# abhi1kumar/SUP-NeRF

Hardware: AMD Instinct MI355X
Metric: rays/sec at 4096 rays x 64 samples (fused render forward) (higher is better)
Workload: dtype f32

## Files before the change

### sup-nerf_amd/csrc/snr_mlp16.hip

```cpp
#include <atomic>

#include "snr_mlp16_core.hpp"
#include "snr_host.hpp"

namespace snr {

struct Epi {
    float lo;
    const float* zlds;
    const float* zglb;
    float hi;
    float* dump;
};
struct EpiRegs { f32x4 z; };

__device__ __forceinline__ uint32_t spread_nibbles(uint32_t m16) {
    return ((m16 >> 12) & 0xFu) | (((m16 >> 8) & 0xFu) << 8) | (((m16 >> 4) & 0xFu) << 16) | ((m16 & 0xFu) << 24);
}

template <bool LATLDS>
__device__ __forceinline__ EpiRegs epi_load(const Epi& c, int T, int g) {
    EpiRegs e;
    e.z = f32x4{0.f, 0.f, 0.f, 0.f};
    if (LATLDS) e.z = *reinterpret_cast<const f32x4*>(c.zlds + 16 * T + 4 * g);
    else if (c.zglb) e.z = *reinterpret_cast<const f32x4*>(c.zglb + 16 * T + 4 * g);
    return e;
}

template <bool MASKS>
__device__ __forceinline__ void epi_value(const f32x4& acc, f32x4& x, const Epi& c, const EpiRegs& e, int r, uint32_t& m16) {
    float v = acc[r];
    if (MASKS) m16 = __builtin_amdgcn_alignbit(m16, __float_as_uint(0.f - v), 31);
    v = __builtin_amdgcn_fmed3f(v, c.lo, c.hi);
    x[r] = v + e.z[r];
    if (MASKS) asm volatile("" : "+v"(m16));
}

template <int NT>
__device__ __forceinline__ void acc_from_bias(f32x4 (&acc)[16], const float* bias , int g) {
#pragma unroll
    for (int t = 0; t < NT; ++t) acc[t] = *reinterpret_cast<const f32x4*>(bias + 16 * t + 4 * g);
}

template <int NT, int WAVES, bool LATLDS, bool MASKS, bool DUMP>
__device__ __forceinline__ void layer_from_acc(f32x4 (&accP)[16], Ring16& ring, float* lds, const float* bias, const Epi& c, int g, const Dma16& dm,
                                               const float* base, bool pre, const f32x4 (&xe)[2], const float* next_first, int next_rows,
                                               uint32_t (&mw)[4]) {
    f32x4 accC[16];
    f32x4 a0, a1;
    constexpr int rows_mid = NT * 16;
    constexpr int chunk_floats = rows_mid * KC;
    if (pre) {
        chunk_dma16<WAVES>(dm, base, lds + (ring.cur ^ 1) * WBUF16, lds, rows_mid);
        const float* wb = lds + ring.cur * WBUF16;
        first_pair(a0, a1, wb + ring.aoff[0]);
        acc_from_bias<NT>(accC, bias, g);
        tile_mma<NT, false>(accC, accP, xe[0], wb + ring.aoff[0], a0, a1, wb + ring.aoff[1]);
        tile_mma<NT, false>(accC, accP, xe[1], wb + ring.aoff[1], a0, a1, nullptr);
        ring_turn(ring);
    } else {
        acc_from_bias<NT>(accC, bias, g);
    }
    constexpr int NG = NT / 2;
    EpiRegs e = epi_load<LATLDS>(c, 0, g);
    f32x4 xa, xb;
    uint32_t m16 = 0u;
#pragma unroll
    for (int r = 3; r >= 0; --r) epi_value<MASKS>(accP[0], xa, c, e, r, m16);
    if (DUMP) *reinterpret_cast<f32x4*>(c.dump) = xa;
#pragma unroll
    for (int ch = 0; ch < 8; ++ch) {
        const float* src = (ch < 7) ? base + (ch + 1) * chunk_floats : next_first;
        const int rows = (ch < 7) ? rows_mid : next_rows;
        float* const dst = lds + (ring.cur ^ 1) * WBUF16;
        const float* wb = lds + ring.cur * WBUF16;
        first_pair(a0, a1, wb + ring.aoff[0]);
        tile_mma<NT, false>(accC, accP, xa, wb + ring.aoff[0], a0, a1, wb + ring.aoff[1], [&](int gi) {
            if (gi == 0) e = epi_load<LATLDS>(c, 2 * ch + 1, g);
            constexpr int PSTEP = (WAVES == 8) ? 2 : 1;
            if (gi % PSTEP == 0 && (gi / PSTEP) * 8 * WAVES < rows) chunk_piece16<WAVES>(dm, src, dst, lds, rows, gi / PSTEP);
#pragma unroll
            for (int k = (gi * 4) / NG; k < ((gi + 1) * 4) / NG; ++k) epi_value<MASKS>(accP[2 * ch + 1], xb, c, e, 3 - k, m16);
            if (DUMP && gi == NG - 1) *reinterpret_cast<f32x4*>(c.dump + 16 * (2 * ch + 1)) = xb;
        });
        if (ch & 1) { mw[ch >> 1] = m16; m16 = 0u; }
        if (ch == 7) {
            tile_mma<NT, true>(accC, accP, xb, wb + ring.aoff[1], a0, a1, nullptr);
        } else {
            tile_mma<NT, false>(accC, accP, xb, wb + ring.aoff[1], a0, a1, nullptr, [&](int gi) {
                if (gi == 0) e = epi_load<LATLDS>(c, 2 * ch + 2, g);
#pragma unroll
                for (int k = (gi * 4) / NG; k < ((gi + 1) * 4) / NG; ++k) epi_value<MASKS>(accP[2 * ch + 2], xa, c, e, 3 - k, m16);
                if (DUMP && gi == NG - 1) *reinterpret_cast<f32x4*>(c.dump + 16 * (2 * ch + 2)) = xa;
            });
        }
        ring_turn(ring);
    }
}

__device__ __forceinline__ void store_masks16x4(uint4* __restrict__ dst , const uint32_t (&mw)[4], int wave, int lane) {
    const int n = lane & 15, g = lane >> 4;
    uint32_t w[4];
#pragma unroll
    for (int i = 0; i < 4; ++i) {
        const uint32_t mine = spread_nibbles(mw[i]) << (4 * (g >> 1));
        w[i] = mine | (uint32_t)__shfl_xor((int)mine, 32, 64);
    }
    if (g < 2) dst[16 * (wave & 1) + n + 32 * g] = make_uint4(w[0], w[1], w[2], w[3]);
}

#ifdef SNR_STAMPS
#define SNR16_STAMP(i) do { if (io.sigmas && lane == 0) { unsigned long long t_; asm volatile("s_memtime %0\n\ts_waitcnt lgkmcnt(0)" : "=s"(t_) :: "memory"); \
        reinterpret_cast<unsigned long long*>(io.sigmas)[(tile_wg * WAVES + wave) * 8 + (i)] = t_; } } while (0)
#define SNR16_STAMP_HWID(i) do { if (io.sigmas && lane == 0) { unsigned a_, b_; asm volatile("s_getreg_b32 %0, hwreg(HW_REG_HW_ID)\n\ts_getreg_b32 %1, hwreg(HW_REG_XCC_ID)" : "=s"(a_), "=s"(b_)); \
        reinterpret_cast<unsigned long long*>(io.sigmas)[(tile_wg * WAVES + wave) * 8 + (i)] = (unsigned long long)a_ | ((unsigned long long)b_ << 32); } } while (0)
#else
#define SNR16_STAMP(i) do {} while (0)
#define SNR16_STAMP_HWID(i) do {} while (0)
#endif

template <int MODE> struct PointSrc { using T = RayGeom; };
template <> struct PointSrc<3> { using T = snr_lattice; };
struct BrickSrc {
    snr_lattice lat;
    const int* bricks;
    long long n_objects;
};
template <> struct PointSrc<4> { using T = BrickSrc; };

template <int MODE, int WAVES, bool LATLDS, bool MASKS, bool DUMP>
__global__ void __launch_bounds__(WAVES * 64, 2)
decoder_fwd16_kernel(DecoderIO io, Layout L, Lds16 lo, const float* __restrict__ xyz, const float* __restrict__ viewdir, typename PointSrc<MODE>::T gm,
                     float* __restrict__ out_rgb, float* __restrict__ out_depth, float* __restrict__ out_acc) {
    extern __shared__ __attribute__((aligned(16))) float lds[];
    constexpr int WGP = WAVES * 16;
    constexpr bool DENS = MODE >= 2;
    const int tid = threadIdx.x, lane = tid & 63, wave = tid >> 6, n = lane & 15, g = lane >> 4;
    const long long tile_wg = blockIdx.x;
    const long long gp_raw = tile_wg * WGP + wave * 16 + n;
    const bool live = gp_raw < io.n_points;
    const long long gp = live ? gp_raw : io.n_points - 1;
    const long long tile32 = tile_wg * (WAVES / 2) + (wave >> 1);
    const bool tile_live = tile32 * 32 < io.n_points;
    const int sb = io.sb, tb = io.tb;
    const int n_relu = n_relu_layers(sb, tb);
    SNR16_STAMP(0);
    __builtin_amdgcn_s_setprio(3);
    float px, py, pz, dx, dy, dz, zc = 0.f;
    long long b_obj = 0, b_dst = 0;
    bool b_keep = false;
    if constexpr (MODE == 0) {
        px = xyz[gp * 3]; py = xyz[gp * 3 + 1]; pz = xyz[gp * 3 + 2];
        dx = viewdir[gp * 3]; dy = viewdir[gp * 3 + 1]; dz = viewdir[gp * 3 + 2];
    } else if constexpr (MODE == 1) {
        const PointId id = point_id(gm, tile_wg, WGP, wave * 16 + n, live);
        const SamplePoint sp = make_sample(gm, id.ray, id.s, id.obj);
        px = sp.x; py = sp.y; pz = sp.z; dx = sp.dx; dy = sp.dy; dz = sp.dz; zc = sp.zc;
    } else if constexpr (MODE == 2) {
        px = xyz[gp * 3]; py = xyz[gp * 3 + 1]; pz = xyz[gp * 3 + 2];
        dx = dy = dz = 0.f;
    } else if constexpr (MODE == 3) {
        const long long obj = gp / io.points_per_obj;
        const unsigned v = (unsigned)(gp - obj * io.points_per_obj), nyz = (unsigned)(gm.n[1] * gm.n[2]);
        const unsigned i = v / nyz, jk = v - i * nyz, j = jk / (unsigned)gm.n[2], k = jk - j * (unsigned)gm.n[2];
        px = gm.lo[0] + gm.h[0] * (float)i; py = gm.lo[1] + gm.h[1] * (float)j; pz = gm.lo[2] + gm.h[2] * (float)k;
        dx = dy = dz = 0.f;
    } else {
        const int* bk = gm.bricks + ((tile_wg * WGP) >> 9) * 4;
        const int nb0 = (gm.lat.n[0] + 7) >> 3, nb1 = (gm.lat.n[1] + 7) >> 3, nb2 = (gm.lat.n[2] + 7) >> 3;
        const bool ok = bk[0] >= 0 && bk[0] < gm.n_objects && bk[1] >= 0 && bk[1] < nb0 && bk[2] >= 0 && bk[2] < nb1 && bk[3] >= 0 && bk[3] < nb2;
        b_obj = ok ? bk[0] : 0;
        const unsigned l = (unsigned)(gp & 511);
        const unsigned i = 8u * (unsigned)(ok ? bk[1] : 0) + (l >> 6), j = 8u * (unsigned)(ok ? bk[2] : 0) + ((l >> 3) & 7u),
                       k = 8u * (unsigned)(ok ? bk[3] : 0) + (l & 7u);
        px = gm.lat.lo[0] + gm.lat.h[0] * (float)i; py = gm.lat.lo[1] + gm.lat.h[1] * (float)j; pz = gm.lat.lo[2] + gm.lat.h[2] * (float)k;
        dx = dy = dz = 0.f;
        b_keep = ok && i < (unsigned)gm.lat.n[0] && j < (unsigned)gm.lat.n[1] && k < (unsigned)gm.lat.n[2];
        b_dst = b_obj * ((long long)gm.lat.n[0] * gm.lat.n[1] * gm.lat.n[2]) + ((long long)i * gm.lat.n[1] + j) * gm.lat.n[2] + k;
    }
    const float* bias = lds + lo.bias;
    const float* heads = bias + L.n_mfma_layers * 256;
    const float* zero = lds + lo.zero;
    const float* lat_lane = io.latent + (MODE == 4 ? b_obj : gp / io.points_per_obj) * (long long)L.n_lat * 256;
    const float* lat_wg = io.latent + (MODE == 4 ? b_obj : (tile_wg * WGP) / io.points_per_obj) * (long long)L.n_lat * 256;

    Ring16 ring;
    ring.cur = 0;
    Dma16 dm;
    dm.voff = lane * 16u + 4096u;
    dm.lds0 = __builtin_amdgcn_readfirstlane((unsigned)(size_t)(__attribute__((address_space(3))) float*)lds);
    dm.wave = __builtin_amdgcn_readfirstlane(wave);
    {
        const int sw = (n >> 1) & 7;
        ring.aoff[0] = n * KC + (((0 + g) ^ sw) << 2);
        ring.aoff[1] = n * KC + (((4 + g) ^ sw) << 2);
    }
    constexpr long long C256 = 256 * KC;
    const int li_encshape = sb + 1, li_view = sb + 2, li_last = sb + tb + 2;
    const float* const stream = io.packed + L.fwd;
    auto layer_base = [&](int li) { return stream + 2 * C256 + (long long)(li - 1) * 8 * C256 + (li > li_view ? C256 : 0); };
    auto layer_first = [&](int li) { return layer_base(li) + (li == li_view ? 8 * C256 : 0); };
    f32x4 xin[4], xd[2];
    {
        chunk_dma16<WAVES>(dm, stream, lds, lds, 256);
        for (int r = dm.wave; r < L.n_mfma_layers + 3; r += WAVES) row_dma16(dm, io.packed + L.bias + r * 256, lds + lo.bias + r * 256, lds);
        if (LATLDS)
            for (int r = dm.wave; r < L.n_lat; r += WAVES) row_dma16(dm, lat_wg + r * 256, lds + lo.lat + r * 256, lds);
        if (tid < 64) *reinterpret_cast<f32x4*>(lds + lo.zero + 4 * tid) = f32x4{0.f, 0.f, 0.f, 0.f};
        float* sc = lds + lo.scratch + wave * PE_WAVE16 + n * PE_ROW;
#pragma unroll 1
        for (int i = 0; i < 8; i += 2) {
            const int q = 8 * g + i;
            if (q < 3 * XYZ_FREQ) {
                f32x2 sn, cs;
                pe_sincos2(f32x2{ldexpf(pick3(px, py, pz, q % 3), q / 3), ldexpf(pick3(px, py, pz, (q + 1) % 3), (q + 1) / 3)}, &sn, &cs);
                sc[3 + q] = sn[0]; sc[3 + 3 * XYZ_FREQ + q] = cs[0];
                sc[4 + q] = sn[1]; sc[4 + 3 * XYZ_FREQ + q] = cs[1];
            }
        }
        if constexpr (!DENS) {
            const int q = 3 * g;
            f32x2 sn, cs;
            pe_sincos2(f32x2{ldexpf(pick3(dx, dy, dz, q % 3), q / 3), ldexpf(pick3(dx, dy, dz, (q + 1) % 3), (q + 1) / 3)}, &sn, &cs);
            sc[64 + 3 + q] = sn[0]; sc[64 + 3 + 3 * DIR_FREQ + q] = cs[0];
            sc[64 + 4 + q] = sn[1]; sc[64 + 4 + 3 * DIR_FREQ + q] = cs[1];
            float s1, c1;
            pe_sincos(ldexpf(pick3(dx, dy, dz, (q + 2) % 3), (q + 2) / 3), &s1, &c1);
            sc[64 + 5 + q] = s1; sc[64 + 5 + 3 * DIR_FREQ + q] = c1;
        }
        if (g == 0) {
            sc[0] = px; sc[1] = py; sc[2] = pz; sc[63] = 0.f;
            if constexpr (!DENS) {
                sc[64] = dx; sc[65] = dy; sc[66] = dz;
#pragma unroll
                for (int f = D_DIR; f < 32; ++f) sc[64 + f] = 0.f;
            }
        }
        asm volatile("s_waitcnt vmcnt(0)" ::: "memory");
        __syncthreads();
#pragma unroll
        for (int T = 0; T < 4; ++T)
#pragma unroll
            for (int r = 0; r < 4; ++r) xin[T][r] = sc[16 * T + 4 * g + r];
#pragma unroll
        for (int T = 0; T < 2; ++T)
#pragma unroll
            for (int r = 0; r < 4; ++r) xd[T][r] = DENS ? 0.f : sc[64 + 16 * T + 4 * g + r];
        if (WAVES == 4) __syncthreads();
    }

    __builtin_amdgcn_s_setprio(0);
    SNR16_STAMP(1);
    f32x4 accP[16];
    {
        f32x4 accC[16];
        f32x4 a0, a1;
        acc_from_bias<16>(accC, bias, g);
#pragma unroll
        for (int ch = 0; ch < 2; ++ch) {
            chunk_dma16<WAVES>(dm, ch == 0 ? stream + C256 : layer_first(1), lds + (ring.cur ^ 1) * WBUF16, lds, 256);
            const float* wb = lds + ring.cur * WBUF16;
            first_pair(a0, a1, wb + ring.aoff[0]);
            tile_mma<16, false>(accC, accP, xin[2 * ch], wb + ring.aoff[0], a0, a1, wb + ring.aoff[1]);
            if (ch == 1) tile_mma<16, true>(accC, accP, xin[2 * ch + 1], wb + ring.aoff[1], a0, a1, nullptr);
            else tile_mma<16, false>(accC, accP, xin[2 * ch + 1], wb + ring.aoff[1], a0, a1, nullptr);
            ring_turn(ring);
        }
    }

    SNR16_STAMP(2);
    uint32_t mw[4] = {0u, 0u, 0u, 0u};
    float o_sigma = 0.f;
    float pos_inf = __builtin_inff();
    asm volatile("" : "+v"(pos_inf));
    float* const dump_lane = DUMP ? io.act + gp * 256 + 4 * g : nullptr;
    auto epi_of = [&](int lp) {
        const int la = latent_after(lp, sb, tb);
        Epi c;
        c.lo = (lp != li_encshape) ? 0.f : -__builtin_inff();
        c.zlds = (la >= 0) ? lds + lo.lat + la * 256 : zero;
        c.zglb = (la >= 0) ? lat_lane + la * 256 : nullptr;
        c.hi = pos_inf;
        c.dump = DUMP ? dump_lane + (long long)lp * io.n_points * 256 : nullptr;
        return c;
    };
    auto after_layer_input = [&](int lp) {
        if (MASKS && lp != li_encshape && tile_live) store_masks16x4(io.masks + (tile32 * n_relu + relu_slot(lp, sb)) * 64, mw, wave, lane);
    };
    const int li_stop = DENS ? li_encshape : li_last;
#pragma unroll 1
    for (int li = 1; li <= li_stop; ++li) {
        const int lp = li - 1;
        const Epi c = epi_of(lp);
        if (!DENS && li == li_view) {
            SNR16_STAMP(3);
            float s = 0.f;
#pragma unroll
            for (int T = 0; T < 16; ++T) {
                const f32x4 ws = *reinterpret_cast<const f32x4*>(heads + 16 * T + 4 * g);
#pragma unroll
                for (int r = 0; r < 4; ++r) s = fmaf(ws[r], accP[T][r], s);
            }
            s += __shfl_xor(s, 16, 64);
            s += __shfl_xor(s, 32, 64);
            const float pre = s + heads[L.sigma_b - L.sigma_w];
            o_sigma = pre > 20.f ? pre : log1pf(expf(pre));
        }
        const bool end = DENS && li == li_stop;
        layer_from_acc<16, WAVES, LATLDS, MASKS, DUMP>(accP, ring, lds, bias + li * 256, c, g, dm, layer_base(li), !DENS && li == li_view, xd,
                                                       end ? nullptr : layer_first(li + 1), end ? 0 : (li == li_last) ? 128 : 256, mw);
        after_layer_input(lp);
    }
    if constexpr (DENS) {
        float s = 0.f;
#pragma unroll
        for (int T = 0; T < 16; ++T) {
            const f32x4 ws = *reinterpret_cast<const f32x4*>(heads + 16 * T + 4 * g);
#pragma unroll
            for (int r = 0; r < 4; ++r) s = fmaf(ws[r], accP[T][r], s);
        }
        s += __shfl_xor(s, 16, 64);
        s += __shfl_xor(s, 32, 64);
        const float pre = s + heads[L.sigma_b - L.sigma_w];
        o_sigma = pre > 20.f ? pre : log1pf(expf(pre));
        if constexpr (MODE == 4) {
            if (b_keep && g == 0) io.sigmas[b_dst] = o_sigma;
        } else {
            if (live && g == 0) io.sigmas[gp] = o_sigma;
        }
        return;
    }
    SNR16_STAMP(4);
    {
        const Epi c = epi_of(li_last);
        layer_from_acc<8, WAVES, LATLDS, MASKS, DUMP>(accP, ring, lds, bias + (li_last + 1) * 256, c, g, dm, layer_base(li_last + 1), false, xd, nullptr, 0, mw);
        after_layer_input(li_last);
    }

    SNR16_STAMP(5);
    __builtin_amdgcn_s_setprio(3);
    float o_r, o_g, o_b;
    {
        const float* w2 = heads + (L.rgb2_w - L.sigma_w);
        float pr = 0.f, pg = 0.f, pb = 0.f;
        uint32_t m16 = 0u, mr[4] = {0u, 0u, 0u, 0u};
        float* const dmp = DUMP ? dump_lane + (long long)(li_last + 1) * io.n_points * 256 : nullptr;
#pragma unroll
        for (int T = 0; T < 8; ++T) {
            const f32x4 wr = *reinterpret_cast<const f32x4*>(w2 + 16 * T + 4 * g);
            const f32x4 wg = *reinterpret_cast<const f32x4*>(w2 + 128 + 16 * T + 4 * g);
            const f32x4 wb = *reinterpret_cast<const f32x4*>(w2 + 256 + 16 * T + 4 * g);
            f32x4 xv;
#pragma unroll
            for (int r = 3; r >= 0; --r) {
                float v = accP[T][r];
                m16 = __builtin_amdgcn_alignbit(m16, __float_as_uint(0.f - v), 31);
                v = fmaxf(v, 0.f);
                xv[r] = v;
            }
#pragma unroll
            for (int r = 0; r < 4; ++r) { pr = fmaf(wr[r], xv[r], pr); pg = fmaf(wg[r], xv[r], pg); pb = fmaf(wb[r], xv[r], pb); }
            if (DUMP) *reinterpret_cast<f32x4*>(dmp + 16 * T) = xv;
            if ((T & 3) == 3) { mr[T >> 2] = m16; m16 = 0u; }
        }
        if (MASKS && tile_live) store_masks16x4(io.masks + (tile32 * n_relu + (n_relu - 1)) * 64, mr, wave, lane);
        pr += __shfl_xor(pr, 16, 64); pr += __shfl_xor(pr, 32, 64);
        pg += __shfl_xor(pg, 16, 64); pg += __shfl_xor(pg, 32, 64);
        pb += __shfl_xor(pb, 16, 64); pb += __shfl_xor(pb, 32, 64);
        const float* b2 = heads + (L.rgb2_b - L.sigma_w);
        o_r = pr + b2[0]; o_g = pg + b2[1]; o_b = pb + b2[2];
    }

    SNR16_STAMP_HWID(6);
#ifndef SNR_STAMPS
    if (live && g == 0 && io.sigmas) io.sigmas[gp] = o_sigma;
#endif
    if (live && g == 0) {
        if (io.rgbs) { io.rgbs[gp * 3] = o_r; io.rgbs[gp * 3 + 1] = o_g; io.rgbs[gp * 3 + 2] = o_b; }
    }
    if constexpr (MODE == 1) {
        float* comp = lds + lo.comp;
        if (g == 0) {
            float* c = comp + (wave * 16 + n) * COMP_STRIDE;
            c[0] = o_sigma; c[1] = o_r; c[2] = o_g; c[3] = o_b; c[4] = zc;
        }
        __syncthreads();
        const int S = gm.S;
        const int rays_here = WGP / S;
        const bool white = gm.flags & SNR_WHITE_BKGD;
        for (int r = wave; r < rays_here; r += WAVES) {
            const long long ray = tile_wg * rays_here + r;
            if (ray >= gm.n_rays) break;
            const float* c0 = comp + r * S * COMP_STRIDE;
            RayOut o = composite_ray_fwd(S, lane, white, [&](int k, float& s_, float& r_, float& g_, float& b_, float& z_, float& zn_) {
                const float* c = c0 + k * COMP_STRIDE;
                s_ = c[0]; r_ = c[1]; g_ = c[2]; b_ = c[3]; z_ = c[4];
                zn_ = (k < S - 1) ? c[COMP_STRIDE + 4] : 0.f;
            });
            if (lane == 0) {
                out_rgb[ray * 3] = o.r; out_rgb[ray * 3 + 1] = o.g; out_rgb[ray * 3 + 2] = o.b;
                out_depth[ray] = o.depth; out_acc[ray] = o.acc;
            }
        }
    }
    SNR16_STAMP(7);
}

}

using namespace snr;


template <int MODE, int WAVES, bool LATLDS, bool MASKS, bool DUMP>
static int launch16(const DecoderIO& io, const Layout& L, const Lds16& lo, const float* xyz, const float* viewdir, const typename PointSrc<MODE>::T& g,
                    float* rgb, float* depth, float* acc, hipStream_t st) {
    auto kern = decoder_fwd16_kernel<MODE, WAVES, LATLDS, MASKS, DUMP>;
    static std::atomic<uint64_t> granted{0};
    int dev = 0;
    if (hipGetDevice(&dev) != hipSuccess) return SNR_E_LAUNCH;
    const uint64_t bit = dev < 64 ? (uint64_t)1 << dev : 0;
    if (!(granted.load(std::memory_order_acquire) & bit)) {
        if (hipFuncSetAttribute(reinterpret_cast<const void*>(kern), hipFuncAttributeMaxDynamicSharedMemorySize, 160 * 1024) != hipSuccess) return SNR_E_LAUNCH;
        granted.fetch_or(bit, std::memory_order_release);
    }
    const unsigned grid = (unsigned)((io.n_points + WAVES * 16 - 1) / (WAVES * 16));
    kern<<<grid, WAVES * 64, (size_t)lo.total * 4, st>>>(io, L, lo, xyz, viewdir, g, rgb, depth, acc);
    return snr_check_launch_();
}

template <int WAVES>
static int launch16_w(int mode, const DecoderIO& io, const Layout& L, const float* xyz, const float* viewdir, const RayGeom& g, float* rgb,
                      float* depth, float* acc, hipStream_t st) {
    const bool latlds = (io.points_per_obj % (WAVES * 16)) == 0 && L.n_lat <= LDS_LAT_ROWS;
    const bool masks = io.masks != nullptr;
    const Lds16 lo = make_lds16(WAVES, L.n_mfma_layers, latlds ? L.n_lat : LDS_LAT_ROWS + 1);
#define SNR_L16(M, LL, MK, DP) launch16<M, WAVES, LL, MK, DP>(io, L, lo, xyz, viewdir, g, rgb, depth, acc, st)
    if (mode == 0) {
        if (latlds) return masks ? SNR_L16(0, true, true, false) : SNR_L16(0, true, false, false);
        return masks ? SNR_L16(0, false, true, false) : SNR_L16(0, false, false, false);
    }
    if (latlds) return masks ? SNR_L16(1, true, true, false) : SNR_L16(1, true, false, false);
    return masks ? SNR_L16(1, false, true, false) : SNR_L16(1, false, false, false);
#undef SNR_L16
}

int snr_fp32_fwd16_launch_(int mode, const DecoderIO& io, const Layout& L, const float* xyz, const float* viewdir, const RayGeom& g, float* rgb,
                           float* depth, float* acc, void* stream_) {
    hipStream_t st = (hipStream_t)stream_;
    if (io.act) return SNR_E_UNSUPPORTED;
    const bool lat4 = (io.points_per_obj % 64) == 0 && L.n_lat <= LDS_LAT_ROWS;
    const Lds16 lo4 = make_lds16(4, L.n_mfma_layers, lat4 ? L.n_lat : LDS_LAT_ROWS + 1);
    const bool four = lo4.total * 4 <= 80 * 1024 && (mode == 0 || (g.S <= 64 && 64 % g.S == 0));
    return four ? launch16_w<4>(mode, io, L, xyz, viewdir, g, rgb, depth, acc, st) : launch16_w<8>(mode, io, L, xyz, viewdir, g, rgb, depth, acc, st);
}

template <int MODE, int WAVES>
static int launch16_dens(const DecoderIO& io, const Layout& L, const float* xyz, const typename PointSrc<MODE>::T& src, hipStream_t st) {
    const bool latlds = (io.points_per_obj % (WAVES * 16)) == 0 && L.n_lat <= LDS_LAT_ROWS;
    const Lds16 lo = make_lds16(WAVES, L.n_mfma_layers, latlds ? L.n_lat : LDS_LAT_ROWS + 1);
    if constexpr (MODE == 2) {
        if (io.masks) {
            if (latlds) return launch16<MODE, WAVES, true, true, false>(io, L, lo, xyz, nullptr, src, nullptr, nullptr, nullptr, st);
            return launch16<MODE, WAVES, false, true, false>(io, L, lo, xyz, nullptr, src, nullptr, nullptr, nullptr, st);
        }
    }
    if (latlds) return launch16<MODE, WAVES, true, false, false>(io, L, lo, xyz, nullptr, src, nullptr, nullptr, nullptr, st);
    return launch16<MODE, WAVES, false, false, false>(io, L, lo, xyz, nullptr, src, nullptr, nullptr, nullptr, st);
}

template <int MODE>
static int density_launch(const DecoderIO& io, const float* xyz, const typename PointSrc<MODE>::T& src, void* stream_) {
    const Layout L = make_layout(io.sb, io.tb);
    const bool lat4 = (io.points_per_obj % 64) == 0 && L.n_lat <= LDS_LAT_ROWS;
    const bool four = make_lds16(4, L.n_mfma_layers, lat4 ? L.n_lat : LDS_LAT_ROWS + 1).total * 4 <= 80 * 1024;
    hipStream_t st = (hipStream_t)stream_;
    return four ? launch16_dens<MODE, 4>(io, L, xyz, src, st) : launch16_dens<MODE, 8>(io, L, xyz, src, st);
}

extern "C" {

int snr_density_fwd(const float* xyz, const float* latent, const float* packed, int64_t n_points, int64_t points_per_obj, int sb, int tb,
                    float* sigmas, void* stream_) {
    if (!xyz || !latent || !packed || !sigmas) return SNR_E_ARG;
    if (sb < 0 || tb < 0 || sb > MAX_BLOCKS || tb > MAX_BLOCKS || n_points < 0) return SNR_E_ARG;
    if (points_per_obj < 1 || (n_points % points_per_obj) != 0) return SNR_E_SHAPE;
    if (n_points == 0) return SNR_OK;
    DecoderIO io{packed, latent, sb, tb, (long long)n_points, (long long)points_per_obj, sigmas, nullptr, nullptr, nullptr, false};
    io.latent_bias = nullptr;
    return density_launch<2>(io, xyz, RayGeom{}, stream_);
}

int snr_density_fwd_masks(const float* xyz, const float* latent, const float* packed, int64_t n_points, int64_t points_per_obj, int sb, int tb,
                          float* sigmas, void* relu_masks, void* stream_) {
    if (!xyz || !latent || !packed || !sigmas || !relu_masks) return SNR_E_ARG;
    if (sb < 0 || tb < 0 || sb > MAX_BLOCKS || tb > MAX_BLOCKS || n_points < 0) return SNR_E_ARG;
    if (points_per_obj < 1 || (n_points % points_per_obj) != 0) return SNR_E_SHAPE;
    if (n_points == 0) return SNR_OK;
    DecoderIO io{packed, latent, sb, tb, (long long)n_points, (long long)points_per_obj, sigmas, nullptr, (uint4*)relu_masks, nullptr, false};
    io.latent_bias = nullptr;
    return density_launch<2>(io, xyz, RayGeom{}, stream_);
}

int snr_density_bricks(const snr_lattice* lattice, int64_t n_objects, const int32_t* bricks, int64_t n_bricks, const float* latent,
                       const float* packed, int sb, int tb, float* sigmas, void* stream_) {
    if (!lattice || !bricks || !latent || !packed || !sigmas) return SNR_E_ARG;
    if (sb < 0 || tb < 0 || sb > MAX_BLOCKS || tb > MAX_BLOCKS || n_objects < 0 || n_bricks < 0) return SNR_E_ARG;
    for (int a = 0; a < 3; ++a)
        if (lattice->n[a] < 1 || lattice->n[a] > 512) return SNR_E_ARG;
    if (n_objects == 0 || n_bricks == 0) return SNR_OK;
    constexpr int64_t CHUNK = 1 << 20;
    for (int64_t off = 0; off < n_bricks; off += CHUNK) {
        const int64_t n = n_bricks - off < CHUNK ? n_bricks - off : CHUNK;
        DecoderIO io{packed, latent, sb, tb, (long long)n * 512, 512, sigmas, nullptr, nullptr, nullptr, false};
        io.latent_bias = nullptr;
        const int rc = density_launch<4>(io, nullptr, BrickSrc{*lattice, bricks + off * 4, (long long)n_objects}, stream_);
        if (rc != SNR_OK) return rc;
    }
    return SNR_OK;
}

int snr_density_grid(const snr_lattice* lattice, int64_t n_objects, const float* latent, const float* packed, int sb, int tb, float* sigmas,
                     void* stream_) {
    if (!lattice || !latent || !packed || !sigmas) return SNR_E_ARG;
    if (sb < 0 || tb < 0 || sb > MAX_BLOCKS || tb > MAX_BLOCKS || n_objects < 0) return SNR_E_ARG;
    for (int a = 0; a < 3; ++a)
        if (lattice->n[a] < 1 || lattice->n[a] > 512) return SNR_E_ARG;
    const long long ppo = (long long)lattice->n[0] * lattice->n[1] * lattice->n[2];
    if (n_objects == 0) return SNR_OK;
    DecoderIO io{packed, latent, sb, tb, (long long)n_objects * ppo, ppo, sigmas, nullptr, nullptr, nullptr, false};
    io.latent_bias = nullptr;
    return density_launch<3>(io, nullptr, *lattice, stream_);
}

}
```

### sup-nerf_amd/csrc/snr_mlp16_core.hpp

```cpp
#pragma once
#include "snr_mlp_core.hpp"

namespace snr {

constexpr int PE_WAVE16 = 16 * PE_ROW;
constexpr int WBUF16 = 256 * KC;

struct Lds16 { int ring1, scratch, comp, bias, lat, zero, total; };
inline Lds16 make_lds16(int waves, int n_mfma_layers, int n_lat) {
    Lds16 o;
    o.ring1 = WBUF16;
    int p = 2 * WBUF16;
    if (waves == 8) { o.scratch = p; p += 8 * PE_WAVE16; o.comp = p; p += 128 * COMP_STRIDE; }
    else { o.scratch = o.ring1; o.comp = 0; }
    p = (p + 3) & ~3;
    o.bias = p; p += (n_mfma_layers + 3) * 256;
    o.lat = p; p += (n_lat <= LDS_LAT_ROWS ? n_lat : 0) * 256;
    o.zero = p; p += 256;
    o.total = p;
    return o;
}

template <int K>
__device__ __forceinline__ void dma_piece_imm(unsigned voff, const void* sbase, unsigned m0v) {
    asm volatile("s_mov_b32 m0, %2\n\ts_nop 0\n\tglobal_load_lds_dwordx4 %0, %1 offset:%3" :: "v"(voff), "s"(sbase), "s"(m0v), "n"(1024 * K - 4096) : "memory");
}
__device__ __forceinline__ void dma_piece(int k, unsigned voff, const void* sbase, unsigned m0v) {
    switch (k) {
        case 0: dma_piece_imm<0>(voff, sbase, m0v); break;
        case 1: dma_piece_imm<1>(voff, sbase, m0v); break;
        case 2: dma_piece_imm<2>(voff, sbase, m0v); break;
        case 3: dma_piece_imm<3>(voff, sbase, m0v); break;
        case 4: dma_piece_imm<4>(voff, sbase, m0v); break;
        case 5: dma_piece_imm<5>(voff, sbase, m0v); break;
        case 6: dma_piece_imm<6>(voff, sbase, m0v); break;
        default: dma_piece_imm<7>(voff, sbase, m0v); break;
    }
}
struct Dma16 {
    unsigned voff;
    unsigned lds0;
    int wave;
};
template <int WAVES>
__device__ __forceinline__ void chunk_piece16(const Dma16& d, const float* __restrict__ g, const float* lds_dst, const float* lds_base, int rows, int i) {
    const unsigned sl = (unsigned)(rows * 128 / WAVES) * (unsigned)d.wave;
    const char* sbase = reinterpret_cast<const char*>(g) + sl;
    const unsigned m0v = __builtin_amdgcn_readfirstlane(d.lds0 + (unsigned)((lds_dst - lds_base) * 4) + sl + 4096u);
    dma_piece(i, d.voff, sbase, m0v);
}
template <int WAVES>
__device__ __forceinline__ void chunk_dma16(const Dma16& d, const float* __restrict__ g, const float* lds_dst, const float* lds_base, int rows) {
#pragma unroll
    for (int i = 0; i < 32 / WAVES; ++i)
        if (i * 8 * WAVES < rows) chunk_piece16<WAVES>(d, g, lds_dst, lds_base, rows, i);
}
__device__ __forceinline__ void row_dma16(const Dma16& d, const float* __restrict__ g, const float* lds_dst, const float* lds_base) {
    const unsigned m0v = __builtin_amdgcn_readfirstlane(d.lds0 + (unsigned)((lds_dst - lds_base) * 4) + 4096u);
    dma_piece_imm<0>(d.voff, g, m0v);
}

struct PointId { long long ray, obj; int s; };
__device__ __forceinline__ PointId point_id(const RayGeom& g, long long tile_wg, int wgp, int pl, bool live) {
    const int ls = 31 - __builtin_clz((unsigned)g.S);
    const long long ray0 = tile_wg * (long long)(wgp >> ls);
    const long long obj0 = ray0 / g.rays_per_obj;
    const long long rem0 = ray0 - obj0 * g.rays_per_obj;
    const int dr = pl >> ls;
    const long long r = rem0 + dr;
    PointId p;
    p.ray = ray0 + dr;
    p.s = pl & (g.S - 1);
    p.obj = obj0 + (g.rays_per_obj >= wgp ? (long long)(r >= g.rays_per_obj) : (long long)((unsigned)r / (unsigned)g.rays_per_obj));
    if (!live) { p.ray = g.n_rays - 1; p.s = g.S - 1; p.obj = (g.n_rays - 1) / g.rays_per_obj; }
    return p;
}

struct Ring16 {
    int cur;
    int aoff[2];
};

#define SNR16_WAIT_LDS() __builtin_amdgcn_s_waitcnt(0xc07f)

struct NoBetween { __device__ __forceinline__ void operator()(int) const {} };
constexpr int TM_LAST = 1, TM_ZERO = 2;
template <int NT, int FLAGS, class Between = NoBetween, int NA = 16, int ND = 16>
__device__ __forceinline__ void tile_mma(f32x4 (&accC)[NA], f32x4 (&accD)[ND], const f32x4& x, const float* wrow ,
                                         f32x4& a0, f32x4& a1, const float* wnext, Between&& between = NoBetween()) {
    constexpr bool LAST = FLAGS & TM_LAST, ZERO = FLAGS & TM_ZERO;
    const f32x4 zero4 = {0.f, 0.f, 0.f, 0.f};
#pragma unroll
    for (int t = 0; t < NT; t += 2) {
        SNR16_WAIT_LDS();
        f32x4 n0 = a0, n1 = a1;
        if (t + 2 < NT) {
            n0 = *reinterpret_cast<const f32x4*>(wrow + (t + 2) * 16 * KC);
            n1 = *reinterpret_cast<const f32x4*>(wrow + (t + 3) * 16 * KC);
        } else if (wnext) {
            n0 = *reinterpret_cast<const f32x4*>(wnext);
            n1 = *reinterpret_cast<const f32x4*>(wnext + 16 * KC);
        }
        __builtin_amdgcn_sched_barrier(0);
#pragma unroll
        for (int r = 0; r < 4; ++r) {
            if (LAST && r == 3) {
                accD[t] = __builtin_amdgcn_mfma_f32_16x16x4f32(a0[r], x[r], accC[t], 0, 0, 0);
                accD[t + 1] = __builtin_amdgcn_mfma_f32_16x16x4f32(a1[r], x[r], accC[t + 1], 0, 0, 0);
            } else {
                accC[t] = __builtin_amdgcn_mfma_f32_16x16x4f32(a0[r], x[r], (ZERO && r == 0) ? zero4 : accC[t], 0, 0, 0);
                accC[t + 1] = __builtin_amdgcn_mfma_f32_16x16x4f32(a1[r], x[r], (ZERO && r == 0) ? zero4 : accC[t + 1], 0, 0, 0);
            }
        }
        between(t / 2);
        __builtin_amdgcn_sched_barrier(0);
        a0 = n0; a1 = n1;
    }
}

__device__ __forceinline__ void first_pair(f32x4& a0, f32x4& a1, const float* wrow) {
    a0 = *reinterpret_cast<const f32x4*>(wrow);
    a1 = *reinterpret_cast<const f32x4*>(wrow + 16 * KC);
}

__device__ __forceinline__ void ring_turn(Ring16& p) {
    asm volatile("s_waitcnt vmcnt(0)" ::: "memory");
    __syncthreads();
    p.cur ^= 1;
}


}
```

Measured before the change: 2.454 million.

## Precompute per-ray view-direction layer contribution once and seed accumulators from LDS

```diff
diff --git a/sup-nerf_amd/csrc/snr_mlp16.hip b/sup-nerf_amd/csrc/snr_mlp16.hip
--- a/sup-nerf_amd/csrc/snr_mlp16.hip
+++ b/sup-nerf_amd/csrc/snr_mlp16.hip
@@ -144,6 +144,10 @@
     const bool tile_live = tile32 * 32 < io.n_points;
     const int sb = io.sb, tb = io.tb;
     const int n_relu = n_relu_layers(sb, tb);
+    const bool seeded = MODE == 1 && lo.seed >= 0;
+    int seed_S = 16;
+    if constexpr (MODE == 1) seed_S = gm.S;
+    const int rays_here = seeded ? WGP / seed_S : 1;
     SNR16_STAMP(0);
     __builtin_amdgcn_s_setprio(3);
     float px, py, pz, dx, dy, dz, zc = 0.f;
@@ -199,9 +203,18 @@
     const int li_encshape = sb + 1, li_view = sb + 2, li_last = sb + tb + 2;
     const float* const stream = io.packed + L.fwd;
     auto layer_base = [&](int li) { return stream + 2 * C256 + (long long)(li - 1) * 8 * C256 + (li > li_view ? C256 : 0); };
-    auto layer_first = [&](int li) { return layer_base(li) + (li == li_view ? 8 * C256 : 0); };
-    f32x4 xin[4], xd[2];
+    auto layer_first = [&](int li) { return layer_base(li) + (li == li_view && !seeded ? 8 * C256 : 0); };
+    auto seed_row = [&](int r) { return r == 0 ? lds + lo.bias + li_view * 256 : lds + lo.seed + (r - 1) * 256; };
+    constexpr int TPW = 16 / WAVES;
+    f32x4 xin[4], xd[2], ad[TPW][2];
     {
+        if (seeded) {
+            const float* dch = layer_base(li_view) + 8 * C256 + (long long)(TPW * wave) * 16 * KC;
+#pragma unroll
+            for (int j = 0; j < TPW; ++j)
+#pragma unroll
+                for (int dT = 0; dT < 2; ++dT) ad[j][dT] = *reinterpret_cast<const f32x4*>(dch + j * 16 * KC + ring.aoff[dT]);
+        }
         chunk_dma16<WAVES>(dm, stream, lds, lds, 256);
         for (int r = dm.wave; r < L.n_mfma_layers + 3; r += WAVES) row_dma16(dm, io.packed + L.bias + r * 256, lds + lo.bias + r * 256, lds);
         if (LATLDS)
@@ -218,7 +231,8 @@
                 sc[4 + q] = sn[1]; sc[4 + 3 * XYZ_FREQ + q] = cs[1];
             }
         }
-        if constexpr (!DENS) {
+        const bool dir_here = !seeded || ((wave * 16) & (seed_S - 1)) == 0;
+        if (!DENS && dir_here) {
             const int q = 3 * g;
             f32x2 sn, cs;
             pe_sincos2(f32x2{ldexpf(pick3(dx, dy, dz, q % 3), q / 3), ldexpf(pick3(dx, dy, dz, (q + 1) % 3), (q + 1) / 3)}, &sn, &cs);
@@ -230,7 +244,7 @@
         }
         if (g == 0) {
             sc[0] = px; sc[1] = py; sc[2] = pz; sc[63] = 0.f;
-            if constexpr (!DENS) {
+            if (!DENS && dir_here) {
                 sc[64] = dx; sc[65] = dy; sc[66] = dz;
 #pragma unroll
                 for (int f = D_DIR; f < 32; ++f) sc[64 + f] = 0.f;
@@ -242,10 +256,23 @@
         for (int T = 0; T < 4; ++T)
 #pragma unroll
             for (int r = 0; r < 4; ++r) xin[T][r] = sc[16 * T + 4 * g + r];
+        const float* dsrc = seeded ? lds + lo.scratch + (n & (rays_here - 1)) * (seed_S >> 4) * PE_WAVE16 + 64 : sc + 64;
 #pragma unroll
         for (int T = 0; T < 2; ++T)
 #pragma unroll
-            for (int r = 0; r < 4; ++r) xd[T][r] = DENS ? 0.f : sc[64 + 16 * T + 4 * g + r];
+            for (int r = 0; r < 4; ++r) xd[T][r] = DENS ? 0.f : dsrc[16 * T + 4 * g + r];
+        if (seeded) {
+#pragma unroll
+            for (int j = 0; j < TPW; ++j) {
+                const int t = TPW * wave + j;
+                f32x4 s = *reinterpret_cast<const f32x4*>(bias + li_view * 256 + 16 * t + 4 * g);
+#pragma unroll
+                for (int dT = 0; dT < 2; ++dT)
+#pragma unroll
+                    for (int r = 0; r < 4; ++r) s = __builtin_amdgcn_mfma_f32_16x16x4f32(ad[j][dT][r], xd[dT][r], s, 0, 0, 0);
+                if (n < rays_here) *reinterpret_cast<f32x4*>(seed_row(n) + 16 * t + 4 * g) = s;
+            }
+        }
         if (WAVES == 4) __syncthreads();
     }
 
@@ -307,7 +334,8 @@
             o_sigma = pre > 20.f ? pre : log1pf(expf(pre));
         }
         const bool end = DENS && li == li_stop;
-        layer_from_acc<16, WAVES, LATLDS, MASKS, DUMP>(accP, ring, lds, bias + li * 256, c, g, dm, layer_base(li), !DENS && li == li_view, xd,
+        const float* start = (seeded && li == li_view) ? seed_row((wave * 16) / seed_S) : bias + li * 256;
+        layer_from_acc<16, WAVES, LATLDS, MASKS, DUMP>(accP, ring, lds, start, c, g, dm, layer_base(li), !DENS && li == li_view && !seeded, xd,
                                                        end ? nullptr : layer_first(li + 1), end ? 0 : (li == li_last) ? 128 : 256, mw);
         after_layer_input(lp);
     }
@@ -433,7 +461,11 @@
                       float* depth, float* acc, hipStream_t st) {
     const bool latlds = (io.points_per_obj % (WAVES * 16)) == 0 && L.n_lat <= LDS_LAT_ROWS;
     const bool masks = io.masks != nullptr;
-    const Lds16 lo = make_lds16(WAVES, L.n_mfma_layers, latlds ? L.n_lat : LDS_LAT_ROWS + 1);
+    Lds16 lo = make_lds16(WAVES, L.n_mfma_layers, latlds ? L.n_lat : LDS_LAT_ROWS + 1);
+    if (mode == 1 && g.S % 16 == 0 && (WAVES * 16) % g.S == 0) {
+        const Lds16 ls = make_lds16(WAVES, L.n_mfma_layers, latlds ? L.n_lat : LDS_LAT_ROWS + 1, WAVES * 16 / g.S - 1);
+        if (ls.total * 4 <= (WAVES == 4 ? 80 : 160) * 1024) lo = ls;
+    }
 #define SNR_L16(M, LL, MK, DP) launch16<M, WAVES, LL, MK, DP>(io, L, lo, xyz, viewdir, g, rgb, depth, acc, st)
     if (mode == 0) {
         if (latlds) return masks ? SNR_L16(0, true, true, false) : SNR_L16(0, true, false, false);
diff --git a/sup-nerf_amd/csrc/snr_mlp16_core.hpp b/sup-nerf_amd/csrc/snr_mlp16_core.hpp
--- a/sup-nerf_amd/csrc/snr_mlp16_core.hpp
+++ b/sup-nerf_amd/csrc/snr_mlp16_core.hpp
@@ -6,8 +6,8 @@
 constexpr int PE_WAVE16 = 16 * PE_ROW;
 constexpr int WBUF16 = 256 * KC;
 
-struct Lds16 { int ring1, scratch, comp, bias, lat, zero, total; };
-inline Lds16 make_lds16(int waves, int n_mfma_layers, int n_lat) {
+struct Lds16 { int ring1, scratch, comp, bias, lat, seed, zero, total; };
+inline Lds16 make_lds16(int waves, int n_mfma_layers, int n_lat, int n_seed = -1) {
     Lds16 o;
     o.ring1 = WBUF16;
     int p = 2 * WBUF16;
@@ -16,6 +16,7 @@
     p = (p + 3) & ~3;
     o.bias = p; p += (n_mfma_layers + 3) * 256;
     o.lat = p; p += (n_lat <= LDS_LAT_ROWS ? n_lat : 0) * 256;
+    o.seed = n_seed >= 0 ? p : -1; p += (n_seed > 0 ? n_seed : 0) * 256;
     o.zero = p; p += 256;
     o.total = p;
     return o;
```

New measurement: 2.476 million, median of 6. Within noise of the previous version (+0.9%).
